# qcraftai/pillarnext

Hardware: AMD Instinct MI355X
Metric: frames/s PillarNeXt-B nuScenes 300k-pt cloud (inference, end-to-end) (higher is better)
Workload: dtype bf16

## Files before the change

pillarnext_amd/csrc/conv3x3.hip:

```cpp
#include "pnx_common.h"

namespace {

typedef float v16f __attribute__((ext_vector_type(16)));
typedef float f32x2 __attribute__((ext_vector_type(2)));

#ifdef PNX_CONV_F16
typedef _Float16 el8 __attribute__((ext_vector_type(8)));
typedef _Float16 el2 __attribute__((ext_vector_type(2)));
#define PNX_MFMA32(a, b, c) __builtin_amdgcn_mfma_f32_32x32x16_f16(a, b, c, 0, 0, 0)
#define PNX_MFMA16(a, b, c) __builtin_amdgcn_mfma_f32_16x16x32_f16(a, b, c, 0, 0, 0)
#define PNX_CONV_FN(name) name##_f16
__device__ __forceinline__ uint32_t el_lo_bits(uint32_t w) { return __float_as_uint((float)__builtin_bit_cast(el2, w)[0]); }
__device__ __forceinline__ uint32_t el_hi_bits(uint32_t w) { return __float_as_uint((float)__builtin_bit_cast(el2, w)[1]); }
#else
typedef __bf16 el8 __attribute__((ext_vector_type(8)));
typedef __bf16 el2 __attribute__((ext_vector_type(2)));
#define PNX_MFMA32(a, b, c) __builtin_amdgcn_mfma_f32_32x32x16_bf16(a, b, c, 0, 0, 0)
#define PNX_MFMA16(a, b, c) __builtin_amdgcn_mfma_f32_16x16x32_bf16(a, b, c, 0, 0, 0)
#define PNX_CONV_FN(name) name##_bf16
__device__ __forceinline__ uint32_t el_lo_bits(uint32_t w) { return w << 16; }
__device__ __forceinline__ uint32_t el_hi_bits(uint32_t w) { return w & 0xffff0000u; }
#endif
__device__ __forceinline__ uint32_t pack_el(float lo, float hi) {
// ... 356 lines not shown
    const int e = part * 256 + tid;
    const int re = e >> 4, ce = 32 + ((e >> 3) & 1);
    if (e < NEXTRA && ((need >> re) & 1u)) {
      uint4 qe = make_uint4(0, 0, 0, 0);
      if (((rows_in >> re) & 1u) && (unsigned)(x0 - 1 + ce) < (unsigned)W)
        qe = *reinterpret_cast<const uint4*>(xt + ((int64_t)re * W + ce) * CSTRIDE + (e & 7) * 8);
      s_in[(re * LDS_HW + ce) * 8 + ((e & 7) ^ lds_swz(ce))] = qe;
    }
  }
}

constexpr int S2_RS = 65;
template <int STRIDE>
__device__ __forceinline__ int tap_slot(int px, int dx) {
  return STRIDE == 1 ? px + dx : (dx == 1 ? px : 32 + px + (dx >> 1));
}
template <int NR, int MTALL, int CB = 4, int STRIDE = 1, int MB = 2>
__device__ __forceinline__ void conv_taps_rolled(v16f (&acc)[NR][MB], const uint4* __restrict__ s_in, const uint4* __restrict__ wfrag, const int (&rbase)[4],
                                          int mg, int px, int kb, int lane, int kstep0 = 0) {
  constexpr int RS = STRIDE == 1 ? LDS_HW : S2_RS;
  uint4 w[4][MB];
#pragma unroll
  for (int cbl = 0; cbl < 4; cbl++)
#pragma unroll
    for (int m = 0; m < MB; m++) w[cbl][m] = wfrag[((kstep0 + cbl) * MTALL + mg + m) * 64 + lane];
#ifdef PNX_CONV_DBG_SAMEW
#define PNX_W_TAP(tn) 0
#else
#define PNX_W_TAP(tn) (tn)
#endif
  uint4 qn[NR];
  {
    const int c0 = tap_slot<STRIDE>(px, 0), sw = lds_swz(c0);
#pragma unroll
    for (int j = 0; j < NR; j++) qn[j] = s_in[rbase[j] + c0 * 8 + (kb ^ sw)];
  }
#pragma unroll 1
  for (int tap = 0; tap < 9; tap++) {
    const int tn = tap + 1;
    const int dyn = tn / 3, dxn = tn - 3 * dyn;
    const int dy = tap / 3, dx = tap - 3 * dy;
    const int c = tap_slot<STRIDE>(px, dx), cn = tap_slot<STRIDE>(px, dxn);
    const int sw = lds_swz(c), swn = lds_swz(cn);
    const int cbase = (dy * RS + c) * 8, cbasen = (dyn * RS + cn) * 8;
#pragma unroll
    for (int cbl = 0; cbl < 4; cbl++) {
      uint4 qc[NR];
#pragma unroll
      for (int j = 0; j < NR; j++) qc[j] = qn[j];
      if (cbl < 3) {
        const int chunk = ((cbl + 1) * 2 + kb) ^ sw;
#pragma unroll
        for (int j = 0; j < NR; j++) qn[j] = s_in[rbase[j] + cbase + chunk];
      } else if (tap < 8) {
        const int chunk = kb ^ swn;
#pragma unroll
        for (int j = 0; j < NR; j++) qn[j] = s_in[rbase[j] + cbasen + chunk];
      }
#pragma unroll
      for (int j = 0; j < NR; j++) {
        const el8 bfr = __builtin_bit_cast(el8, qc[j]);
#pragma unroll
        for (int m = 0; m < MB; m++)
          acc[j][m] = PNX_MFMA32(__builtin_bit_cast(el8, w[cbl][m]), bfr, acc[j][m]);
      }
      if (tap < 8) {
#pragma unroll
        for (int m = 0; m < MB; m++) w[cbl][m] = wfrag[((PNX_W_TAP(tn) * CB + kstep0 + cbl) * MTALL + mg + m) * 64 + lane];
      }
      __builtin_amdgcn_sched_barrier(0);
    }
  }
}

#ifndef TAPS_PD
#define TAPS_PD 1
#endif
#ifndef TAPS_WD
#define TAPS_WD 4
#endif
#ifndef TAPS_NOBUFW
#define TAPS_BUFW
#endif
template <int NR, int MTALL, int CB = 4, int STRIDE = 1, int MB = 2, int WD = TAPS_WD>
__device__ __forceinline__ void conv_taps(v16f (&acc)[NR][MB], const uint4* __restrict__ s_in, const uint4* __restrict__ wfrag, const int (&rbase)[4],
                                          int mg, int px, int kb, int lane, int kstep0 = 0) {
#ifdef PNX_TAPS_ROLLED
  conv_taps_rolled<NR, MTALL, CB, STRIDE, MB>(acc, s_in, wfrag, rbase, mg, px, kb, lane, kstep0);
#else
  constexpr int RS = STRIDE == 1 ? LDS_HW : S2_RS;
  constexpr int KS = 36, PD = TAPS_PD;
  const uint4* wu = wfrag + (int64_t)__builtin_amdgcn_readfirstlane(kstep0 * MTALL + mg) * 64;
#ifdef TAPS_BUFW
  const __amdgpu_buffer_rsrc_t wrs = __builtin_amdgcn_make_buffer_rsrc(const_cast<uint4*>(wu), 0, 0x7fffffff, 0x00020000);
  const int wlo = lane * 16;
#endif
  auto wload = [&](int ks, uint4 (&dst)[MB]) {
    const int grp = ks / 3, cbl = grp & 3;
#ifdef PNX_CONV_DBG_SAMEW
    const int tap = 0;
#else
    const int tap = (ks % 3) * 3 + (grp >> 2);
#endif
#pragma unroll
    for (int m = 0; m < MB; m++) {
#ifdef TAPS_BUFW
      typedef unsigned int u32x4 __attribute__((ext_vector_type(4)));
      const u32x4 r = __builtin_amdgcn_raw_buffer_load_b128(wrs, wlo, (((tap * CB + cbl) * MTALL + m) * 64) * 16, 0);
      dst[m] = make_uint4(r.x, r.y, r.z, r.w);
#else
      dst[m] = wu[((tap * CB + cbl) * MTALL + m) * 64 + lane];
#endif
    }
  };
  int addr[NR];
  auto group_addr = [&](int grp) {
    const int dx = grp >> 2, cbl = grp & 3;
    int p = px;
    asm volatile("" : "+v"(p));
    const int c = tap_slot<STRIDE>(p, dx);
    const int a = c * 8 + ((2 * cbl + kb) ^ lds_swz(c));
#pragma unroll
    for (int j = 0; j < NR; j++) addr[j] = a + rbase[j];
  };
  auto bload = [&](int ks, uint4 (&dst)[NR]) {
    const int dy = ks % 3;
    if (dy == 0) group_addr(ks / 3);
#pragma unroll
    for (int j = 0; j < NR; j++) dst[j] = s_in[addr[j] + dy * (RS * 8)];
  };
  uint4 w[WD][MB];
  uint4 q[PD + 1][NR];
#pragma unroll
  for (int k = 0; k < WD; k++) wload(k, w[k]);
#pragma unroll
  for (int k = 0; k < PD; k++) bload(k, q[k]);
#pragma unroll
  for (int ks = 0; ks < KS; ks++) {
    if (ks + PD < KS) bload(ks + PD, q[(ks + PD) % (PD + 1)]);
#pragma unroll
    for (int j = 0; j < NR; j++) {
      const el8 bfr = __builtin_bit_cast(el8, q[ks % (PD + 1)][j]);
#pragma unroll
      for (int m = 0; m < MB; m++) acc[j][m] = PNX_MFMA32(__builtin_bit_cast(el8, w[ks % WD][m]), bfr, acc[j][m]);
    }
    if (ks + WD < KS) wload(ks + WD, w[ks % WD]);
#ifndef TAPS_NOSB
    __builtin_amdgcn_sched_barrier(0);
#endif
  }
#endif
}

template <int NR, int COUT, bool HAS_RES>
__device__ __forceinline__ void conv_rows(const uint4* __restrict__ s_in, const uint4* __restrict__ wfrag, const float* __restrict__ bias,
                                          const uint16_t* const (&rrow_res)[4], uint32_t res_off, const int (&rbase)[4], const uint32_t (&rmask)[4],
                                          uint16_t* const (&yrow)[4], int n_valid, int relu, int px, int kb, int lane) {
  constexpr int MTALL = COUT / 32;
#pragma unroll 1
  for (int mg = 0; mg < MTALL; mg += 2) {
    v16f acc[NR][2];
#pragma unroll
    for (int m = 0; m < 2; m++) {
      const v16f bq = bias_tile(bias, (mg + m) * 32, kb);
#pragma unroll
      for (int j = 0; j < NR; j++) acc[j][m] = bq;
    }
#ifdef PNX_CONV_RES_EARLY
    if (HAS_RES) {
#pragma unroll
      for (int j = 0; j < NR; j++) {
        uint4 rq[2][2];
        load_residual_u(rq, rrow_res[j], res_off, (rmask[j] >> px) & 1u);
        add_residual(acc[j], rq);
      }
    }
#endif
    uint4 rq[2][2];
#ifndef PNX_CONV_RES_EARLY
    if (HAS_RES) load_residual_u(rq, rrow_res[0], res_off, rmask[0] >> px & 1u);
#endif
    conv_taps<NR, MTALL, 4, 1, 2, COUT == 64 ? 2 : TAPS_WD>(acc, s_in, wfrag, rbase, mg, px, kb, lane);
#pragma unroll
    for (int j = 0; j < NR; j++) {
      const bool act = (rmask[j] >> px) & 1u;
      uint4 rc[2][2];
#ifndef PNX_CONV_RES_EARLY
      if (HAS_RES) {
#pragma unroll
        for (int m = 0; m < 2; m++)
#pragma unroll
          for (int t = 0; t < 2; t++) rc[m][t] = rq[m][t];
        if (j + 1 < NR) load_residual_u(rq, rrow_res[j + 1], res_off, rmask[j + 1] >> px & 1u);
      }
#endif
      uint4 D[4];
#pragma unroll
      for (int m = 0; m < 2; m++) {
        uint4 pk[2];
#ifndef PNX_CONV_RES_EARLY
// ... 146 lines not shown
__device__ __forceinline__ void conv_rows_x(uint4* __restrict__ s_in, const uint16_t* __restrict__ x, const uint4* __restrict__ wfrag,
                                            const float* __restrict__ bias, const uint16_t* __restrict__ res, const int (&rrow)[4],
                                            const int (&rbase)[4], const uint32_t (&rmask)[4], uint16_t* const (&yrow)[4], int b, int H, int W,
                                            int y0, int x0, uint32_t need, int mg0, int relu, int px, int kb, int lane, int hsel) {
  constexpr int NS = CIN / 64, NRA = NR > 0 ? NR : 1;
  const int ox = x0 + px;
  {
    const int h = hsel;
    const int mg = mg0 + 4 * h;
    v16f acc[NRA][2];
    if (NR > 0) {
#pragma unroll
      for (int m = 0; m < 2; m++) {
        const v16f bq = bias_tile(bias, (mg + m) * 32, kb);
#pragma unroll
        for (int j = 0; j < NR; j++) acc[j][m] = bq;
      }
#ifdef PNX_CONV_RES_EARLY
      if (HAS_RES) {
#pragma unroll
        for (int j = 0; j < NR; j++) {
          uint4 rq[2][2];
          load_residual_u(rq, res + (((int64_t)b * H + (y0 + rrow[j])) * W + x0) * COUT + mg * 32, (uint32_t)(px * COUT + 8 * kb) * 2u, (rmask[j] >> px) & 1u);
          add_residual(acc[j], rq);
        }
      }
#endif
    }
    const uint16_t* rres[NRA];
    const uint32_t res_off = (uint32_t)(px * COUT + 8 * kb) * 2u;
    uint4 rq[2][2];
    if (NR > 0 && HAS_RES) {
#pragma unroll
      for (int j = 0; j < NR; j++) rres[j] = res + (((int64_t)b * H + (y0 + rrow[j])) * W + x0) * COUT + mg * 32;
    }
#pragma unroll 1
    for (int sl = 0; sl < NS; sl++) {
      if (sl) {
        __syncthreads();
        stage_tile64<CIN, L128_TH>(s_in, x, b, H, W, 64 * sl, y0, x0, need);
        __syncthreads();
      }
#ifndef PNX_CONV_RES_EARLY
      if (NR > 0 && HAS_RES && sl == NS - 1) load_residual_u(rq, rres[0], res_off, rmask[0] >> px & 1u);
#endif
#ifndef LDSX_RES_WD
#define LDSX_RES_WD 2
#endif
      if (NR > 0) conv_taps<NRA, COUT / 32, CIN / 16, 1, 2, HAS_RES ? LDSX_RES_WD : TAPS_WD>(acc, s_in, wfrag, rbase, mg, px, kb, lane, 4 * sl);
    }
    if (NR > 0) {
      const int n_valid = W - x0;
#pragma unroll
      for (int j = 0; j < NR; j++) {
        const bool act = (rmask[j] >> px) & 1u;
        uint4 rc[2][2];
#ifndef PNX_CONV_RES_EARLY
        if (HAS_RES) {
#pragma unroll
          for (int m = 0; m < 2; m++)
#pragma unroll
            for (int t = 0; t < 2; t++) rc[m][t] = rq[m][t];
          if (j + 1 < NR) load_residual_u(rq, rres[j + 1], res_off, rmask[j + 1] >> px & 1u);
        }
#endif
        uint4 D[4];
#pragma unroll
        for (int m = 0; m < 2; m++) {
          uint4 pk[2];
#ifndef PNX_CONV_RES_EARLY
          pack_tile(acc[j][m], act, relu, pk, HAS_RES ? rc[m] : nullptr);
#else
          pack_tile(acc[j][m], act, relu, pk);
#endif
          D[2 * m] = pk[0], D[2 * m + 1] = pk[1];
        }
        transpose_row64(D, lane);
        store_row64<COUT>(D, yrow[j] + mg * 32, n_valid, lane);
      }
    }
  }
}

template <int CIN, int COUT, bool HAS_RES>
__global__ __launch_bounds__(256, 2) void k_conv3x3_ldsx(const uint16_t* __restrict__ x, const uint4* __restrict__ wfrag,
                                                      const float* __restrict__ bias, const uint16_t* __restrict__ res,
                                                      const uint8_t* __restrict__ mask, uint16_t* __restrict__ y, int B, int H, int W,
                                                      int relu, uint8_t* __restrict__ row_dirty, int slot, const int32_t* __restrict__ tlist,
                                                      const int32_t* __restrict__ tcount) {
  static_assert(CIN % 64 == 0 && (COUT % 128 == 0 || COUT == 64), "64-channel input slabs, 128-channel output passes (or one of 64)");
  constexpr int TH = L128_TH, HW_ = LDS_HW;
  constexpr int NRG = COUT == 64 ? 4 : 2, NRMAX = TH / NRG;
  __shared__ uint4 s_in[L128_NSTAGE];
  __shared__ uint32_t s_rowmask2[2 * TH];
  __shared__ unsigned int s_next[2];
  const int lane = threadIdx.x & 63, wv = threadIdx.x >> 6;
  const int px = lane & 31, kb = lane >> 5;
  const int rg = wv % NRG, mg0 = 2 * (wv / NRG);
  const int tiles_x = (W + 31) >> 5, tiles_y = (H + TH - 1) / TH;
  const int n_tiles = tlist != nullptr ? __builtin_amdgcn_readfirstlane(*tcount) : B * tiles_y * tiles_x;
  constexpr int NH = (COUT + 127) / 128;
  const int n_units = n_tiles * NH;
  auto unit_at = [&](int64_t idx) -> int {
    if (idx >= n_units) return -1;
    const int i = (int)idx;
    const int t = tlist != nullptr ? tlist[i / NH] : i / NH;
    return t * NH + i % NH;
  };
  auto load_mask = [&](int t, bool (&a)[2], int (&wz)[2]) {
#pragma unroll
    for (int j = 0; j < 2; j++) a[j] = false, wz[j] = 1;
    if (t < 0) return;
    const int tx = (int)(t % tiles_x);
    const int ty = (int)((t / tiles_x) % tiles_y);
    const int b = (int)(t / ((int64_t)tiles_x * tiles_y));
    const int ox = tx * 32 + px;
#pragma unroll
    for (int j = 0; j < 2; j++) {
      const int oy = ty * TH + wv * 2 + j;
      a[j] = ox < W && oy < H && (mask == nullptr || mask[((int64_t)b * H + oy) * W + ox] != 0);
      if (row_dirty != nullptr && oy < H) wz[j] = (int)row_dirty[((int64_t)b * H + oy) * tiles_x + tx];
    }
  };
  int64_t idxB = (int64_t)blockIdx.x + gridDim.x, idxC = 0;
  int tileA = unit_at(blockIdx.x), tileB = unit_at(idxB), tileC = -1;
  bool aP[2], aN[2];
  int wasP[2], wasN[2];
  load_mask(tileA >= 0 ? tileA / NH : -1, aP, wasP);
#pragma unroll
  for (int j = 0; j < 2; j++) aN[j] = false, wasN[j] = 1;
  int it = 0;
  for (; tileA >= 0; tileA = tileB, tileB = tileC, idxB = idxC, it++) {
    const int unit = __builtin_amdgcn_readfirstlane(tileA);
    const int tile = unit / NH;
    const int hsel = unit - tile * NH;
    sched_draw(s_next, it, slot);
    uint32_t* const s_rowmask = s_rowmask2 + (it & 1) * TH;
    const int tx = (int)(tile % tiles_x);
    const int ty = (int)((tile / tiles_x) % tiles_y);
    const int b = (int)(tile / ((int64_t)tiles_x * tiles_y));
    const int x0 = tx * 32, y0 = ty * TH;
    const int ox = x0 + px;
    bool was[2];
#pragma unroll
    for (int j = 0; j < 2; j++) {
      was[j] = __builtin_amdgcn_readfirstlane(wasP[j]) != 0;
      const uint32_t bal = (uint32_t)__ballot(aP[j]);
      if (lane == 0) s_rowmask[wv * 2 + j] = bal;
    }
    __syncthreads();
    idxC = sched_next2(s_next, it, slot, idxB);
    tileC = unit_at(idxC);
    load_mask(tileB >= 0 ? tileB / NH : -1, aN, wasN);
#pragma unroll
    for (int j = 0; j < 2; j++) aP[j] = aN[j], wasP[j] = wasN[j];
    const uint32_t my_rm = s_rowmask[lane & 7];
    const uint32_t am = (uint32_t)__ballot(my_rm != 0) & 0xffu;
#pragma unroll
    for (int j = 0; j < 2; j++) {
      const int rr = wv * 2 + j, oy = y0 + rr;
      const bool active = (am >> rr) & 1u;
      if (hsel != 0) continue;
      if (!active && was[j] && oy < H && ox < W) {
        uint4* dst = reinterpret_cast<uint4*>(y + (((int64_t)b * H + oy) * W + ox) * COUT);
#pragma unroll 1
        for (int ch = kb; ch < COUT / 8; ch += 2) dst[ch] = make_uint4(0, 0, 0, 0);
      }
      if (row_dirty != nullptr && oy < H && lane == 0 && was[j] != active) row_dirty[((int64_t)b * H + oy) * tiles_x + tx] = active ? 1 : 0;
    }
    if (am == 0) continue;
    int nr = 0;
    int rbase[4], rrow[4];
    {
      uint32_t rest = am;
      for (int k = 0; k < rg && rest; k++) rest &= rest - 1;
#pragma unroll
      for (int j = 0; j < 4; j++) {
        const bool has = j < NRMAX && rest != 0;
        rrow[j] = has ? __builtin_ctz(rest) : 0;
        nr += has ? 1 : 0;
        for (int k = 0; k < NRG && rest; k++) rest &= rest - 1;
      }
    }
    nr = __builtin_amdgcn_readfirstlane(nr);
    uint32_t rmask[4];
    uint16_t* yrow[4];
#pragma unroll
    for (int j = 0; j < 4; j++) {
      rrow[j] = __builtin_amdgcn_readfirstlane(rrow[j]);
      rbase[j] = rrow[j] * HW_ * 8;
      rmask[j] = j < nr ? __builtin_amdgcn_readfirstlane(s_rowmask[rrow[j]]) : 0u;
      yrow[j] = y + (((int64_t)b * H + (y0 + rrow[j])) * W + x0) * COUT;
    }
    const uint32_t need = am | (am << 1) | (am << 2);
    stage_tile64<CIN, TH>(s_in, x, b, H, W, 0, y0, x0, need);
    __syncthreads();
#define PNX_ROWS_X(N_) conv_rows_x<(N_ <= NRMAX ? N_ : NRMAX), CIN, COUT, HAS_RES>(s_in, x, wfrag, bias, res, rrow, rbase, rmask, yrow, b, H, W, y0, x0, need, mg0, relu, px, kb, lane, hsel)
    switch (nr) {
      case 0: PNX_ROWS_X(0); break;
      case 1: PNX_ROWS_X(1); break;
      case 2: PNX_ROWS_X(2); break;
      case 3: PNX_ROWS_X(3); break;
      default: PNX_ROWS_X(4); break;
    }
#undef PNX_ROWS_X
  }
  sched_done(slot);
}

template <int CIN, int COUT>
int launch_ldsx(const void* x, const void* wfrag, const float* bias, const void* res, const uint8_t* mask, void* y, int B, int H, int W, int relu,
                uint8_t* row_dirty, const int32_t* tlist, const int32_t* tcount, hipStream_t st) {
  const int slot = mask != nullptr ? next_sched_slot() : -1;
  int64_t nb = (int64_t)B * ((H + L128_TH - 1) / L128_TH) * ((W + 31) / 32) * ((COUT + 127) / 128);
  if (nb > 512) nb = 512;
  if (res != nullptr)
    k_conv3x3_ldsx<CIN, COUT, true><<<(unsigned)nb, 256, 0, st>>>((const uint16_t*)x, (const uint4*)wfrag, bias, (const uint16_t*)res, mask, (uint16_t*)y,
                                                                 B, H, W, relu, row_dirty, slot, tlist, tcount);
  else
    k_conv3x3_ldsx<CIN, COUT, false><<<(unsigned)nb, 256, 0, st>>>((const uint16_t*)x, (const uint4*)wfrag, bias, nullptr, mask, (uint16_t*)y, B, H, W,
                                                                  relu, row_dirty, slot, tlist, tcount);
  PNX_LAUNCH_CHECK();
  return PNX_OK;
}

constexpr int S2_TH = 4;
constexpr int S2_ROWS = 2 * S2_TH + 1;
constexpr int S2_NSTAGE = S2_ROWS * S2_RS * 8;

template <int CSTRIDE>
__device__ __forceinline__ void stage_tile64_s2(uint4* __restrict__ s_in, const uint16_t* __restrict__ x, int b, int H, int W, int ch0, int iy0,
                                                int ix0, uint32_t need) {
  typedef __attribute__((address_space(1))) const void* gptr_t;
  typedef __attribute__((address_space(3))) void* lptr_t;
  int tid = threadIdx.x;
  asm volatile("" : "+v"(tid));
  const int slot = tid & 7, col = tid >> 3, wbase = (tid >> 6) * 8;
  const uint16_t* xb = x + (int64_t)b * H * W * CSTRIDE + ch0;
#pragma unroll
  for (int pl = 0; pl < 2; pl++) {
    const int ls = pl * 32 + col;
    const int ix = ix0 + 2 * col + (1 - pl);
    const bool col_ok = (unsigned)ix < (unsigned)W;
    const int chunk = slot ^ lds_swz(ls);
#pragma unroll
    for (int r = 0; r < S2_ROWS; r++) {
      if (!((need >> r) & 1u)) continue;
      const int iy = iy0 + r;
      if ((unsigned)iy < (unsigned)H && col_ok) {
        __builtin_amdgcn_global_load_lds((gptr_t)(xb + ((int64_t)iy * W + ix) * CSTRIDE + chunk * 8),
                                         (lptr_t)(s_in + (r * S2_RS + pl * 32 + wbase) * 8), 16, 0, 0);
      } else {
        s_in[(r * S2_RS + ls) * 8 + slot] = make_uint4(0, 0, 0, 0);
      }
    }
  }
  if (tid < S2_ROWS * 8) {
    const int re = tid >> 3, ce = tid & 7;
    if ((need >> re) & 1u) {
      const int iy = iy0 + re, ix = ix0 + 64;
      uint4 qe = make_uint4(0, 0, 0, 0);
      if ((unsigned)iy < (unsigned)H && (unsigned)ix < (unsigned)W) qe = *reinterpret_cast<const uint4*>(xb + ((int64_t)iy * W + ix) * CSTRIDE + ce * 8);
      s_in[(re * S2_RS + 64) * 8 + (ce ^ lds_swz(64))] = qe;
    }
  }
}

template <int NR, int CIN, int COUT, int MB, int NP = 1>
__device__ __forceinline__ void conv_rows_s2(uint4* __restrict__ s_in, const uint16_t* __restrict__ x, const uint16_t* __restrict__ x2,
                                             const uint16_t* __restrict__ x3, const uint4* __restrict__ wfrag, const uint4* __restrict__ wfrag2,
                                             const uint4* __restrict__ wfrag3, const float* __restrict__ bias, const int (&rbase)[4], const uint32_t (&rmask)[4],
                                             uint16_t* const (&yrow)[4], int b, int H, int W, int iy0, int ix0, int n_valid, uint32_t need, int mg,
                                             int relu, int px, int kb, int lane) {
  constexpr int NS = CIN / 64, NRA = NR > 0 ? NR : 1;
  constexpr bool X3 = NP == 2, F32 = NP > 1;
  v16f acc[NRA][MB];
  if (NR > 0) {
#pragma unroll
    for (int m = 0; m < MB; m++) {
      v16f bq;
      if (F32 && bias == nullptr) {
#pragma unroll
        for (int i = 0; i < 16; i++) bq[i] = 0.f;
      } else {
        bq = bias_tile(bias, (mg + m) * 32, kb);
      }
#pragma unroll
      for (int j = 0; j < NR; j++) acc[j][m] = bq;
    }
  }
#pragma unroll 1
  for (int sq = 0; sq < NS * NP; sq++) {
    const int sl = F32 ? sq % NS : sq;
    if (sq) {
      __syncthreads();
      const uint16_t* xs = X3 && sq >= NS ? x2 : x;
      if constexpr (NP == 3) xs = sq < NS ? x3 : sq < 2 * NS ? x2 : x;
      stage_tile64_s2<CIN>(s_in, xs, b, H, W, 64 * sl, iy0, ix0, need);
// ... 408 lines not shown
    default: break;
  }
  pnx_set_error("pnx_sephead_out: no kernel for %d branches", n_branch);
  return PNX_ERR_UNSUPPORTED;
}

int PNX_CONV_FN(pnx_deconv2x2)(const void* x, const void* wfrag, const float* bias, void* y, int32_t batch, int32_t h, int32_t w, int32_t cin, int32_t cout,
                       int32_t relu, pnx_stream_t stream) {
  PNX_REQUIRE(x && wfrag && bias && y && batch > 0 && h > 0 && w > 0, PNX_ERR_INVALID, "bad arguments");
  PNX_REQUIRE((((uintptr_t)x | (uintptr_t)y | (uintptr_t)wfrag | (uintptr_t)bias) & 15) == 0, PNX_ERR_INVALID, "16-byte alignment required");
  if (cin != 64 || cout != 64) {
    pnx_set_error("pnx_deconv2x2: no kernel for %d -> %d channels", cin, cout);
    return PNX_ERR_UNSUPPORTED;
  }
  const int64_t n_seg = (int64_t)batch * h * ((w + 31) / 32);
  int64_t nb = (n_seg + 3) / 4;
  if (nb > 512) nb = 512;
  k_deconv2x2_64<<<(unsigned)nb, 256, 0, (hipStream_t)stream>>>((const uint16_t*)x, (const uint4*)wfrag, bias, (uint16_t*)y, batch, h, w, relu);
  PNX_LAUNCH_CHECK();
  return PNX_OK;
}

#ifndef PNX_CONV_F16
int pnx_conv3x3_tile_rows(int32_t cin, int32_t cout, int32_t stride) {
  if (stride != 1) return 0;
  if (cin == 64 && (cout == 64 || cout == 320 || cout == 384 || cout == 448)) return LDS_TH;
  if ((cin == 128 && cout == 128) || (cin == 256 && (cout == 256 || cout == 64))) return L128_TH;
  return 0;
}

static int conv_tile_list_impl(const uint8_t* mask, const uint8_t* const* row_dirty, int32_t n_dirty, int32_t batch, int32_t h, int32_t w, int32_t tile_rows,
                               int32_t* tile_list, int32_t* tile_count, pnx_stream_t stream, bool zero_count) {
  PNX_REQUIRE(mask && tile_list && tile_count && batch > 0 && h > 0 && w > 0 && tile_rows > 0, PNX_ERR_INVALID, "bad arguments");
  PNX_REQUIRE(n_dirty >= 0 && n_dirty <= 4 && (n_dirty == 0 || row_dirty != nullptr), PNX_ERR_INVALID, "0..4 row_dirty arrays");
  DirtySet ds;
  for (int k = 0; k < 4; k++) ds.p[k] = k < n_dirty ? row_dirty[k] : nullptr;
  hipStream_t st = (hipStream_t)stream;
  if (zero_count) PNX_CHECK_HIP(hipMemsetAsync(tile_count, 0, sizeof(int32_t), st));
  const int64_t n_tiles = (int64_t)batch * ((h + tile_rows - 1) / tile_rows) * ((w + 31) / 32);
  PNX_REQUIRE(tile_rows <= 16, PNX_ERR_UNSUPPORTED, "tile_rows %d (at most 16: one lane per row)", tile_rows);
  k_tile_list<<<(unsigned)((n_tiles + 15) / 16), 256, 0, st>>>(mask, ds, batch, h, w, tile_rows, tile_list, tile_count);
  PNX_LAUNCH_CHECK();
  return PNX_OK;
}
int pnx_conv_tile_list(const uint8_t* mask, const uint8_t* const* row_dirty, int32_t n_dirty, int32_t batch, int32_t h, int32_t w, int32_t tile_rows,
                       int32_t* tile_list, int32_t* tile_count, pnx_stream_t stream) {
  return conv_tile_list_impl(mask, row_dirty, n_dirty, batch, h, w, tile_rows, tile_list, tile_count, stream, true);
}
int pnx_conv_tile_list_prezeroed(const uint8_t* mask, const uint8_t* const* row_dirty, int32_t n_dirty, int32_t batch, int32_t h, int32_t w, int32_t tile_rows,
                                 int32_t* tile_list, int32_t* tile_count, pnx_stream_t stream) {
  return conv_tile_list_impl(mask, row_dirty, n_dirty, batch, h, w, tile_rows, tile_list, tile_count, stream, false);
}

#endif

int PNX_CONV_FN(pnx_conv3x3)(const void* x, const void* wfrag, const float* bias, const void* residual, const uint8_t* mask, void* y, int32_t batch,
                     int32_t h, int32_t w, int32_t cin, int32_t cout, int32_t stride, int32_t relu, uint8_t* row_dirty, const int32_t* tile_list,
                     const int32_t* tile_count, pnx_stream_t stream) {
  PNX_REQUIRE((tile_list == nullptr) == (tile_count == nullptr), PNX_ERR_INVALID, "tile_list and tile_count come together");
  PNX_REQUIRE(tile_list == nullptr || (mask != nullptr && pnx_conv3x3_tile_rows(cin, cout, stride) > 0), PNX_ERR_INVALID,
              "a tile list needs a mask and a kernel that takes one (pnx_conv3x3_tile_rows)");
  PNX_REQUIRE(x && wfrag && bias && y && batch > 0 && h > 0 && w > 0, PNX_ERR_INVALID, "bad arguments");
  PNX_REQUIRE(stride == 1 || stride == 2, PNX_ERR_UNSUPPORTED, "stride %d", stride);
  PNX_REQUIRE(row_dirty == nullptr || mask != nullptr, PNX_ERR_INVALID, "row_dirty needs an active-site mask");
  PNX_REQUIRE((((uintptr_t)x | (uintptr_t)y | (uintptr_t)wfrag | (uintptr_t)bias | (uintptr_t)residual) & 15) == 0, PNX_ERR_INVALID,
              "16-byte alignment required");
  const int ho = (h + 2 - 3) / stride + 1, wo = (w + 2 - 3) / stride + 1;
  hipStream_t st = (hipStream_t)stream;
  if (stride == 1 && getenv("PNX_CONV_DIRECT") == nullptr) {
    static const int pc_mode = getenv("PNX_CONV_PC") != nullptr ? atoi(getenv("PNX_CONV_PC")) : 1;
    if (pc_mode != 0) {
      if (cin == 64 && cout == 64) return launch_pc<64, 64>(x, wfrag, bias, residual, mask, y, batch, h, w, relu, row_dirty, tile_list, tile_count, st);
      if (residual == nullptr && (pc_mode & 4)) {
        if (cin == 64 && cout == 320) return launch_pc<64, 320>(x, wfrag, bias, residual, mask, y, batch, h, w, relu, row_dirty, tile_list, tile_count, st);
        if (cin == 64 && cout == 384) return launch_pc<64, 384>(x, wfrag, bias, residual, mask, y, batch, h, w, relu, row_dirty, tile_list, tile_count, st);
        if (cin == 64 && cout == 448) return launch_pc<64, 448>(x, wfrag, bias, residual, mask, y, batch, h, w, relu, row_dirty, tile_list, tile_count, st);
      }
      if (pc_mode & 2) {
        if (cin == 128 && cout == 128) return launch_pc<128, 128>(x, wfrag, bias, residual, mask, y, batch, h, w, relu, row_dirty, tile_list, tile_count, st);
        if (cin == 256 && cout == 256) return launch_pc<256, 256>(x, wfrag, bias, residual, mask, y, batch, h, w, relu, row_dirty, tile_list, tile_count, st);
      }
    }
    if (cin == 64 && cout == 64) return launch_lds<64>(x, wfrag, bias, residual, mask, y, batch, h, w, relu, row_dirty, tile_list, tile_count, st);
    if (cin == 128 && cout == 128) return launch_ldsx<128, 128>(x, wfrag, bias, residual, mask, y, batch, h, w, relu, row_dirty, tile_list, tile_count, st);
    if (cin == 256 && cout == 64) return launch_ldsx<256, 64>(x, wfrag, bias, residual, mask, y, batch, h, w, relu, row_dirty, tile_list, tile_count, st);
    if (cin == 256 && cout == 256) return launch_ldsx<256, 256>(x, wfrag, bias, residual, mask, y, batch, h, w, relu, row_dirty, tile_list, tile_count, st);
    if (cin == 64 && cout == 384) return launch_lds<384>(x, wfrag, bias, residual, mask, y, batch, h, w, relu, row_dirty, tile_list, tile_count, st);
    if (cin == 64 && cout == 320) return launch_lds<320>(x, wfrag, bias, residual, mask, y, batch, h, w, relu, row_dirty, tile_list, tile_count, st);
    if (cin == 64 && cout == 448) return launch_lds<448>(x, wfrag, bias, residual, mask, y, batch, h, w, relu, row_dirty, tile_list, tile_count, st);
  }
  if (stride == 2 && residual == nullptr && getenv("PNX_CONV_DIRECT") == nullptr) {
    if (cin == 64 && cout == 128) return launch_s2<64, 128>(x, wfrag, bias, mask, y, batch, h, w, ho, wo, relu, row_dirty, st);
    if (cin == 128 && cout == 256) return launch_s2<128, 256>(x, wfrag, bias, mask, y, batch, h, w, ho, wo, relu, row_dirty, st);
    if (cin == 256 && cout == 256) return launch_s2<256, 256>(x, wfrag, bias, mask, y, batch, h, w, ho, wo, relu, row_dirty, st);
  }
#define PNX_CONV_CASE(CI, CO)                                                                                          \
  if (cin == CI && cout == CO) {                                                                                       \
    if (stride == 1) return launch<CI, CO, 1>(x, wfrag, bias, residual, mask, y, batch, h, w, ho, wo, relu, row_dirty, st);         \
    return launch<CI, CO, 2>(x, wfrag, bias, residual, mask, y, batch, h, w, ho, wo, relu, row_dirty, st);                         \
  }
  PNX_CONV_CASE(64, 64)
  PNX_CONV_CASE(64, 128)
  PNX_CONV_CASE(128, 128)
#undef PNX_CONV_CASE
  pnx_set_error("pnx_conv3x3: no kernel for %d -> %d channels", cin, cout);
  return PNX_ERR_UNSUPPORTED;
}

#ifndef PNX_CONV_F16
}
namespace {
#include "conv_dgrad_s2.h"
}
extern "C" {

int pnx_conv3x3_dgrad_s2_bf16(const void* g, const void* wfrag_t, const uint8_t* mask_in, void* dx, int32_t batch, int32_t h, int32_t w, int32_t cin, int32_t cout,
                              pnx_stream_t stream) {
  PNX_REQUIRE(g && wfrag_t && mask_in && dx && batch > 0 && h > 0 && w > 0, PNX_ERR_INVALID, "pnx_conv3x3_dgrad_s2_bf16: bad arguments");
  PNX_REQUIRE((((uintptr_t)g | (uintptr_t)wfrag_t | (uintptr_t)dx) & 15) == 0, PNX_ERR_INVALID, "16-byte alignment required");
  hipStream_t st = (hipStream_t)stream;
  if (cin == 64 && cout == 128) return launch_dgrad_s2<128, 64, 1>(g, nullptr, wfrag_t, nullptr, mask_in, dx, batch, h, w, st);
  if (cin == 128 && cout == 256) return launch_dgrad_s2<256, 128, 1>(g, nullptr, wfrag_t, nullptr, mask_in, dx, batch, h, w, st);
  if (cin == 256 && cout == 256) return launch_dgrad_s2<256, 256, 1>(g, nullptr, wfrag_t, nullptr, mask_in, dx, batch, h, w, st);
  pnx_set_error("pnx_conv3x3_dgrad_s2_bf16: no kernel for %d -> %d channels", cin, cout);
  return PNX_ERR_UNSUPPORTED;
}

int pnx_conv3x3_dgrad_s2_x3(const void* g_hi, const void* g_lo, const void* wfrag_t_hi, const void* wfrag_t_lo, const uint8_t* mask_in, float* dx, int32_t batch,
                            int32_t h, int32_t w, int32_t cin, int32_t cout, pnx_stream_t stream) {
  PNX_REQUIRE(g_hi && g_lo && wfrag_t_hi && wfrag_t_lo && mask_in && dx && batch > 0 && h > 0 && w > 0, PNX_ERR_INVALID, "pnx_conv3x3_dgrad_s2_x3: bad arguments");
  PNX_REQUIRE((((uintptr_t)g_hi | (uintptr_t)g_lo | (uintptr_t)wfrag_t_hi | (uintptr_t)wfrag_t_lo | (uintptr_t)dx) & 15) == 0, PNX_ERR_INVALID,
              "16-byte alignment required");
  hipStream_t st = (hipStream_t)stream;
  if (cin == 64 && cout == 128) return launch_dgrad_s2<128, 64, 2>(g_hi, g_lo, wfrag_t_hi, wfrag_t_lo, mask_in, dx, batch, h, w, st);
  if (cin == 128 && cout == 256) return launch_dgrad_s2<256, 128, 2>(g_hi, g_lo, wfrag_t_hi, wfrag_t_lo, mask_in, dx, batch, h, w, st);
  if (cin == 256 && cout == 256) return launch_dgrad_s2<256, 256, 2>(g_hi, g_lo, wfrag_t_hi, wfrag_t_lo, mask_in, dx, batch, h, w, st);
  pnx_set_error("pnx_conv3x3_dgrad_s2_x3: no kernel for %d -> %d channels", cin, cout);
  return PNX_ERR_UNSUPPORTED;
}

int pnx_conv3x3_dgrad_s2_x6(const void* g_hi, const void* g_mid, const void* g_lo, const void* wfrag_t_hi, const void* wfrag_t_mid, const void* wfrag_t_lo,
                            const uint8_t* mask_in, float* dx, int32_t batch, int32_t h, int32_t w, int32_t cin, int32_t cout, pnx_stream_t stream) {
  PNX_REQUIRE(g_hi && g_mid && g_lo && wfrag_t_hi && wfrag_t_mid && wfrag_t_lo && mask_in && dx && batch > 0 && h > 0 && w > 0, PNX_ERR_INVALID,
              "pnx_conv3x3_dgrad_s2_x6: bad arguments");
  PNX_REQUIRE((((uintptr_t)g_hi | (uintptr_t)g_mid | (uintptr_t)g_lo | (uintptr_t)wfrag_t_hi | (uintptr_t)wfrag_t_mid | (uintptr_t)wfrag_t_lo | (uintptr_t)dx) & 15) == 0,
              PNX_ERR_INVALID, "16-byte alignment required");
  hipStream_t st = (hipStream_t)stream;
  if (cin == 64 && cout == 128) return launch_dgrad_s2<128, 64, 3>(g_hi, g_mid, wfrag_t_hi, wfrag_t_mid, mask_in, dx, batch, h, w, st, g_lo, wfrag_t_lo);
  if (cin == 128 && cout == 256) return launch_dgrad_s2<256, 128, 3>(g_hi, g_mid, wfrag_t_hi, wfrag_t_mid, mask_in, dx, batch, h, w, st, g_lo, wfrag_t_lo);
  if (cin == 256 && cout == 256) return launch_dgrad_s2<256, 256, 3>(g_hi, g_mid, wfrag_t_hi, wfrag_t_mid, mask_in, dx, batch, h, w, st, g_lo, wfrag_t_lo);
  pnx_set_error("pnx_conv3x3_dgrad_s2_x6: no kernel for %d -> %d channels", cin, cout);
  return PNX_ERR_UNSUPPORTED;
}

int pnx_conv3x3_x3(const void* x_hi, const void* x_lo, const void* wfrag_hi, const void* wfrag_lo, const float* bias, const uint8_t* mask, float* y,
                   int32_t batch, int32_t h, int32_t w, int32_t cin, int32_t cout, int32_t stride, pnx_stream_t stream) {
  PNX_REQUIRE(x_hi && x_lo && wfrag_hi && wfrag_lo && y, PNX_ERR_INVALID, "null pointer");
  PNX_REQUIRE(batch > 0 && h > 0 && w > 0, PNX_ERR_INVALID, "bad shape");
  PNX_REQUIRE(stride == 1 || stride == 2, PNX_ERR_UNSUPPORTED, "stride %d", stride);
  PNX_REQUIRE((((uintptr_t)x_hi | (uintptr_t)x_lo | (uintptr_t)y | (uintptr_t)wfrag_hi | (uintptr_t)wfrag_lo | (uintptr_t)bias) & 15) == 0, PNX_ERR_INVALID,
              "16-byte alignment required");
  hipStream_t st = (hipStream_t)stream;
  if (stride == 1) {
    if (cin == 64 && cout == 64) return launch_pc_x3<64, 64>(x_hi, x_lo, wfrag_hi, wfrag_lo, bias, mask, y, batch, h, w, st);
    if (cin == 128 && cout == 128) return launch_pc_x3<128, 128>(x_hi, x_lo, wfrag_hi, wfrag_lo, bias, mask, y, batch, h, w, st);
    if (cin == 256 && cout == 256) return launch_pc_x3<256, 256>(x_hi, x_lo, wfrag_hi, wfrag_lo, bias, mask, y, batch, h, w, st);
  } else {
    const int ho = (h - 1) / 2 + 1, wo = (w - 1) / 2 + 1;
    if (cin == 64 && cout == 128) return launch_s2<64, 128, 2>(x_hi, wfrag_hi, bias, mask, y, batch, h, w, ho, wo, 0, nullptr, st, x_lo, wfrag_lo);
// ... 244 lines not shown
```

Measured before the change: 705.9.

## Pack active pixels into dense 32-wide groups for 128/256-channel sparse 3x3 conv

Adds a packed-pixel variant of the LDS-staged 3x3 conv kernel for the 128->128 and 256->256 layers. Active pixels of a tile are compacted into a shared list and processed in dense groups of 32, with per-pixel LDS addressing and scattered stores, instead of row-by-row with idle lanes. Inactive pixels that were previously active are explicitly zeroed. The aim is fewer MFMA passes on sparse tiles, at the cost of extra bookkeeping, packed-code address computation and scattered output writes. It is enabled by default and can be turned off with an environment variable.

```diff
diff --git a/pillarnext_amd/csrc/conv3x3.hip b/pillarnext_amd/csrc/conv3x3.hip
--- a/pillarnext_amd/csrc/conv3x3.hip
+++ b/pillarnext_amd/csrc/conv3x3.hip
@@ -462,10 +462,11 @@
 #ifndef TAPS_NOBUFW
 #define TAPS_BUFW
 #endif
-template <int NR, int MTALL, int CB = 4, int STRIDE = 1, int MB = 2, int WD = TAPS_WD>
+template <int NR, int MTALL, int CB = 4, int STRIDE = 1, int MB = 2, int WD = TAPS_WD, bool PIX = false>
 __device__ __forceinline__ void conv_taps(v16f (&acc)[NR][MB], const uint4* __restrict__ s_in, const uint4* __restrict__ wfrag, const int (&rbase)[4],
                                           int mg, int px, int kb, int lane, int kstep0 = 0) {
 #ifdef PNX_TAPS_ROLLED
+  static_assert(!PIX, "the rolled tap loop has no packed-pixel form");
   conv_taps_rolled<NR, MTALL, CB, STRIDE, MB>(acc, s_in, wfrag, rbase, mg, px, kb, lane, kstep0);
 #else
   constexpr int RS = STRIDE == 1 ? LDS_HW : S2_RS;
@@ -496,6 +497,18 @@
   int addr[NR];
   auto group_addr = [&](int grp) {
     const int dx = grp >> 2, cbl = grp & 3;
+    if constexpr (PIX) {
+      int p = rbase[0];
+      asm volatile("" : "+v"(p));
+#pragma unroll
+      for (int j = 0; j < NR; j++) {
+        const int q = (p >> (8 * j)) & 255;
+        const int c = tap_slot<STRIDE>(q & 31, dx);
+        addr[j] = (q >> 5) * (RS * 8) + c * 8 + ((2 * cbl + kb) ^ lds_swz(c));
+        asm volatile("" : "+v"(addr[j]));
+      }
+      return;
+    }
     int p = px;
     asm volatile("" : "+v"(p));
     const int c = tap_slot<STRIDE>(p, dx);
@@ -808,7 +821,79 @@
   }
 }
 
-template <int CIN, int COUT, bool HAS_RES>
+__device__ __forceinline__ int pix_code(int row, int col) { return (row << 5) | col; }
+template <int CSTRIDE>
+__device__ __forceinline__ uint32_t pix_off(int code, int W) { return (uint32_t)(((code >> 5) * W + (code & 31)) * CSTRIDE) * 2u; }
+
+template <int CSTRIDE>
+__device__ __forceinline__ void store_pix64(const uint4 (&D)[4], uint16_t* __restrict__ tile, int code, int n_valid, int W, int lane) {
+  int l = lane;
+  asm volatile("" : "+v"(l));
+#pragma unroll
+  for (int d = 0; d < 4; d++) {
+    const int P = 8 * d + (l >> 3);
+    const int pc = __builtin_amdgcn_ds_bpermute(P << 2, code);
+    if (P < n_valid) *reinterpret_cast<uint4*>(reinterpret_cast<char*>(tile) + pix_off<CSTRIDE>(pc, W) + (uint32_t)((l & 7) * 16)) = D[d];
+  }
+}
+
+template <int NR, int CIN, int COUT, bool HAS_RES>
+__device__ __forceinline__ void conv_pix_x(uint4* __restrict__ s_in, const uint16_t* __restrict__ x, const uint4* __restrict__ wfrag,
+                                           const float* __restrict__ bias, const uint16_t* __restrict__ rtile, int codes, const int (&n_g)[4],
+                                           uint16_t* __restrict__ ytile, int b, int H, int W, int y0, int x0, uint32_t need, int mg0, int relu, int px,
+                                           int kb, int lane, int hsel) {
+  constexpr int NS = CIN / 64, NRA = NR > 0 ? NR : 1;
+  const int mg = mg0 + 4 * hsel;
+  v16f acc[NRA][2];
+  if (NR > 0) {
+#pragma unroll
+    for (int m = 0; m < 2; m++) {
+      const v16f bq = bias_tile(bias, (mg + m) * 32, kb);
+#pragma unroll
+      for (int j = 0; j < NR; j++) acc[j][m] = bq;
+    }
+  }
+  const uint16_t* const rres = HAS_RES ? rtile + mg * 32 : nullptr;
+  auto code = [&](int j) { return (codes >> (8 * j)) & 255; };
+  auto res_off = [&](int j) { return pix_off<COUT>(code(j), W) + (uint32_t)(16 * kb); };
+  const int cw[4] = {codes, 0, 0, 0};
+  uint4 rq[2][2];
+#pragma unroll 1
+  for (int sl = 0; sl < NS; sl++) {
+    if (sl) {
+      __syncthreads();
+      stage_tile64<CIN, L128_TH>(s_in, x, b, H, W, 64 * sl, y0, x0, need);
+      __syncthreads();
+    }
+    if (NR > 0 && HAS_RES && sl == NS - 1) load_residual_u(rq, rres, res_off(0), px < n_g[0]);
+    if (NR > 0) conv_taps<NRA, COUT / 32, CIN / 16, 1, 2, HAS_RES ? LDSX_RES_WD : TAPS_WD, true>(acc, s_in, wfrag, cw, mg, px, kb, lane, 4 * sl);
+  }
+  if (NR > 0) {
+#pragma unroll
+    for (int j = 0; j < NR; j++) {
+      const bool act = px < n_g[j];
+      uint4 rc[2][2];
+      if (HAS_RES) {
+#pragma unroll
+        for (int m = 0; m < 2; m++)
+#pragma unroll
+          for (int t = 0; t < 2; t++) rc[m][t] = rq[m][t];
+        if (j + 1 < NR) load_residual_u(rq, rres, res_off(j + 1), px < n_g[j + 1]);
+      }
+      uint4 D[4];
+#pragma unroll
+      for (int m = 0; m < 2; m++) {
+        uint4 pk[2];
+        pack_tile(acc[j][m], act, relu, pk, HAS_RES ? rc[m] : nullptr);
+        D[2 * m] = pk[0], D[2 * m + 1] = pk[1];
+      }
+      transpose_row64(D, lane);
+      store_pix64<COUT>(D, ytile + mg * 32, code(j), n_g[j], W, lane);
+    }
+  }
+}
+
+template <int CIN, int COUT, bool HAS_RES, bool PACK = false>
 __global__ __launch_bounds__(256, 2) void k_conv3x3_ldsx(const uint16_t* __restrict__ x, const uint4* __restrict__ wfrag,
                                                       const float* __restrict__ bias, const uint16_t* __restrict__ res,
                                                       const uint8_t* __restrict__ mask, uint16_t* __restrict__ y, int B, int H, int W,
@@ -817,7 +902,9 @@
   static_assert(CIN % 64 == 0 && (COUT % 128 == 0 || COUT == 64), "64-channel input slabs, 128-channel output passes (or one of 64)");
   constexpr int TH = L128_TH, HW_ = LDS_HW;
   constexpr int NRG = COUT == 64 ? 4 : 2, NRMAX = TH / NRG;
+  static_assert(!PACK || (CIN == COUT && NRG == 2), "the packed-pixel form serves 128 -> 128 and 256 -> 256");
   __shared__ uint4 s_in[L128_NSTAGE];
+  __shared__ uint16_t s_list[PACK ? TH * 32 : 1];
   __shared__ uint32_t s_rowmask2[2 * TH];
   __shared__ unsigned int s_next[2];
   const int lane = threadIdx.x & 63, wv = threadIdx.x >> 6;
@@ -868,11 +955,12 @@
     const int x0 = tx * 32, y0 = ty * TH;
     const int ox = x0 + px;
     bool was[2];
+    uint32_t bal[2];
 #pragma unroll
     for (int j = 0; j < 2; j++) {
       was[j] = __builtin_amdgcn_readfirstlane(wasP[j]) != 0;
-      const uint32_t bal = (uint32_t)__ballot(aP[j]);
-      if (lane == 0) s_rowmask[wv * 2 + j] = bal;
+      bal[j] = (uint32_t)__ballot(aP[j]);
+      if (lane == 0) s_rowmask[wv * 2 + j] = bal[j];
     }
     __syncthreads();
     idxC = sched_next2(s_next, it, slot, idxB);
@@ -895,6 +983,60 @@
       if (row_dirty != nullptr && oy < H && lane == 0 && was[j] != active) row_dirty[((int64_t)b * H + oy) * tiles_x + tx] = active ? 1 : 0;
     }
     if (am == 0) continue;
+    if constexpr (PACK) {
+      const int wvu = __builtin_amdgcn_readfirstlane(wv);
+      int n_px = 0, pos = 0;
+#pragma unroll
+      for (int k = 0; k < TH; k++) {
+        const int n = __builtin_popcount(__builtin_amdgcn_readlane(my_rm, k));
+        n_px += n;
+        pos += k < 2 * wvu ? n : 0;
+      }
+#pragma unroll
+      for (int j = 0; j < 2; j++) {
+        if (kb == 0 && ((bal[j] >> px) & 1u)) s_list[pos + __builtin_popcount(bal[j] & ((1u << px) - 1u))] = (uint16_t)pix_code(wvu * 2 + j, px);
+        pos += __builtin_popcount(bal[j]);
+      }
+      const int n_grp = (n_px + 31) >> 5, rgu = __builtin_amdgcn_readfirstlane(rg);
+      const int nr = n_grp > rgu ? (n_grp - rgu + 1) >> 1 : 0;
+      const uint32_t need = am | (am << 1) | (am << 2);
+      stage_tile64<CIN, TH>(s_in, x, b, H, W, 0, y0, x0, need);
+      __syncthreads();
+      int codes = 0, n_g[4];
+#pragma unroll
+      for (int j = 0; j < 4; j++) {
+        const int g = rgu + 2 * j;
+        n_g[j] = min(max(n_px - 32 * g, 0), 32);
+        if (j < nr && px < n_g[j]) codes |= (int)s_list[32 * g + px] << (8 * j);
+      }
+      const int64_t t0 = (((int64_t)b * H + y0) * W + x0) * COUT;
+#define PNX_PIX_X(N_) conv_pix_x<N_, CIN, COUT, HAS_RES>(s_in, x, wfrag, bias, HAS_RES ? res + t0 : nullptr, codes, n_g, y + t0, b, H, W, y0, x0, need, mg0, relu, px, kb, lane, hsel)
+      switch (nr) {
+        case 0: PNX_PIX_X(0); break;
+        case 1: PNX_PIX_X(1); break;
+        case 2: PNX_PIX_X(2); break;
+        case 3: PNX_PIX_X(3); break;
+        default: PNX_PIX_X(4); break;
+      }
+#undef PNX_PIX_X
+      int l = lane;
+      asm volatile("" : "+v"(l));
+      const uint32_t cols = W - x0 >= 32 ? 0xffffffffu : (1u << (W - x0)) - 1u;
+#pragma unroll
+      for (int j = 0; j < 2; j++) {
+        const int rr = wvu * 2 + j;
+        const uint32_t idle = ~bal[j] & cols;
+        if (!((am >> rr) & 1u) || !was[j] || y0 + rr >= H || idle == 0) continue;
+        char* const row = reinterpret_cast<char*>(y + t0) + (uint32_t)(rr * W * COUT * 2 + hsel * 256);
+#pragma unroll 1
+        for (int c0 = 0; c0 < 32; c0 += 4) {
+          if (((idle >> c0) & 15u) == 0) continue;
+          const int p = c0 + (l >> 4);
+          if ((idle >> p) & 1u) *reinterpret_cast<uint4*>(row + (uint32_t)(p * COUT * 2 + (l & 15) * 16)) = make_uint4(0, 0, 0, 0);
+        }
+      }
+      continue;
+    }
     int nr = 0;
     int rbase[4], rrow[4];
     {
@@ -936,10 +1078,22 @@
 
 template <int CIN, int COUT>
 int launch_ldsx(const void* x, const void* wfrag, const float* bias, const void* res, const uint8_t* mask, void* y, int B, int H, int W, int relu,
-                uint8_t* row_dirty, const int32_t* tlist, const int32_t* tcount, hipStream_t st) {
+                uint8_t* row_dirty, const int32_t* tlist, const int32_t* tcount, hipStream_t st, bool pack = false) {
   const int slot = mask != nullptr ? next_sched_slot() : -1;
   int64_t nb = (int64_t)B * ((H + L128_TH - 1) / L128_TH) * ((W + 31) / 32) * ((COUT + 127) / 128);
   if (nb > 512) nb = 512;
+  if constexpr (CIN == COUT) {
+    if (pack && mask != nullptr) {
+      if (res != nullptr)
+        k_conv3x3_ldsx<CIN, COUT, true, true><<<(unsigned)nb, 256, 0, st>>>((const uint16_t*)x, (const uint4*)wfrag, bias, (const uint16_t*)res, mask,
+                                                                          (uint16_t*)y, B, H, W, relu, row_dirty, slot, tlist, tcount);
+      else
+        k_conv3x3_ldsx<CIN, COUT, false, true><<<(unsigned)nb, 256, 0, st>>>((const uint16_t*)x, (const uint4*)wfrag, bias, nullptr, mask, (uint16_t*)y, B, H,
+                                                                           W, relu, row_dirty, slot, tlist, tcount);
+      PNX_LAUNCH_CHECK();
+      return PNX_OK;
+    }
+  }
   if (res != nullptr)
     k_conv3x3_ldsx<CIN, COUT, true><<<(unsigned)nb, 256, 0, st>>>((const uint16_t*)x, (const uint4*)wfrag, bias, (const uint16_t*)res, mask, (uint16_t*)y,
                                                                  B, H, W, relu, row_dirty, slot, tlist, tcount);
@@ -1514,9 +1668,10 @@
       }
     }
     if (cin == 64 && cout == 64) return launch_lds<64>(x, wfrag, bias, residual, mask, y, batch, h, w, relu, row_dirty, tile_list, tile_count, st);
-    if (cin == 128 && cout == 128) return launch_ldsx<128, 128>(x, wfrag, bias, residual, mask, y, batch, h, w, relu, row_dirty, tile_list, tile_count, st);
+    static const bool pack = getenv("PNX_CONV_PACK") == nullptr || atoi(getenv("PNX_CONV_PACK")) != 0;
+    if (cin == 128 && cout == 128) return launch_ldsx<128, 128>(x, wfrag, bias, residual, mask, y, batch, h, w, relu, row_dirty, tile_list, tile_count, st, pack);
     if (cin == 256 && cout == 64) return launch_ldsx<256, 64>(x, wfrag, bias, residual, mask, y, batch, h, w, relu, row_dirty, tile_list, tile_count, st);
-    if (cin == 256 && cout == 256) return launch_ldsx<256, 256>(x, wfrag, bias, residual, mask, y, batch, h, w, relu, row_dirty, tile_list, tile_count, st);
+    if (cin == 256 && cout == 256) return launch_ldsx<256, 256>(x, wfrag, bias, residual, mask, y, batch, h, w, relu, row_dirty, tile_list, tile_count, st, pack);
     if (cin == 64 && cout == 384) return launch_lds<384>(x, wfrag, bias, residual, mask, y, batch, h, w, relu, row_dirty, tile_list, tile_count, st);
     if (cin == 64 && cout == 320) return launch_lds<320>(x, wfrag, bias, residual, mask, y, batch, h, w, relu, row_dirty, tile_list, tile_count, st);
     if (cin == 64 && cout == 448) return launch_lds<448>(x, wfrag, bias, residual, mask, y, batch, h, w, relu, row_dirty, tile_list, tile_count, st);
```

After: 749.9 (median of 6 runs). 6.2% higher.
